# sashajenner/honours

Hardware: AMD Instinct MI355X
Metric: raw-signal MB/s (compress+decompress) (higher is better)
Workload: dtype u16

## Files before the change

honours_amd/csrc/press_abi.hip:

```cpp

#include <dlfcn.h>
#include <stdarg.h>
#include <stdio.h>
#include <stdlib.h>
#include <string.h>

#include <mutex>
#include <thread>
#include <algorithm>
#include <vector>

#include "../../include/press_hip.h"
#include "press_internal.h"
#include "zs_table.h"

using namespace ph;


static thread_local char g_err[256] = "";

static int fail(int code, const char *fmt, ...)
{
	va_list ap;
	va_start(ap, fmt);
// ... 24 lines not shown
	DevBuf() : next(g_bufs) { g_bufs = this; }
	DevBuf(const DevBuf &) = delete;
	DevBuf &operator=(const DevBuf &) = delete;
	int reserve(size_t n)
	{
		if (n <= cap)
			return 0;
		if (p)
			(void) hipFree(p);
		p = nullptr;
		cap = 0;
		size_t want = n + n / 8 + 4096;
		hipError_t e = hipMalloc(&p, want);
		if (e != hipSuccess)
			return fail(PRESS_HIP_EHIP, "hipMalloc(%zu): %s", want, hipGetErrorString(e));
		cap = want;
		return 0;
	}
	void release()
	{
		if (p)
			(void) hipFree(p);
		p = nullptr;
		cap = 0;
	}
};

struct Ctx {
	bool ready = false;
	int device = -1;
	hipStream_t own = nullptr;
	hipStream_t user = nullptr;
	bool use_user = false;
	DevBuf meta, ex_pos, ex_val, low, huff, chunks, gran, ctl, first_chunk, htiles, htrec, hrec, hlist, hread, hwave, hbits, hend, hmin, cbits;
	DevBuf ztmp, zoff, zoff4, zlen, zhist, ztab, zfirst, zblk, zsbits, zbpos, zbflag, zkcnt, zrd, znb, zn, zdcopy, zdhuf, zdunit, zdtree, zdlong, zdctl, zdseq, zdxblk;
	DevBuf sig, off, nsamp, arena, arena_off, lens, lens2, outn, dense, dense_off;
	uint64_t zs_total = 0;
	uint32_t zs_nhost = 0;
	uint32_t *zs_pin = nullptr;
	hipEvent_t zs_ev = nullptr;
	bool have_table = false;
	bool table_trie = false;
	uint32_t tlen[256];
	uint64_t tbits[256];

	hipStream_t stream() const { return use_user ? user : own; }
};

Ctx g;
std::recursive_mutex g_mu;
#define API_LOCK std::lock_guard<std::recursive_mutex> api_lock_(g_mu)
void staging_release();

int ctx_init()
{
	if (g.ready) {
		HIPCHK(hipSetDevice(g.device));
		return 0;
	}
	int ndev = 0;
	hipError_t e = hipGetDeviceCount(&ndev);
	if (e != hipSuccess || ndev == 0)
		return fail(PRESS_HIP_EHIP, "no HIP device: %s", hipGetErrorString(e));
	if (g.device < 0)
		HIPCHK(hipGetDevice(&g.device));
	HIPCHK(hipSetDevice(g.device));
	HIPCHK(hipStreamCreateWithFlags(&g.own, hipStreamNonBlocking));
// ... 333 lines not shown
		    g.zdctl.reserve(sizeof(ZsDCtl)))
			return PRESS_HIP_EHIP;
	}
	if (is_zs(method) && !decode) {
		const size_t mc = max_chunks_of(total_samples, nreads), mb = max_zblocks_of(total_samples, nreads);
		const size_t nr = (size_t) nreads + 1;
		if (g.ztmp.reserve(zs_tmp_bytes(method, total_samples, nreads)) || g.zoff.reserve(nr * 8) || g.zoff4.reserve(nr * 8) ||
		    g.zlen.reserve(nr * 8) || g.zhist.reserve(nr * 1024) || g.ztab.reserve(nr * sizeof(zs::Table)) ||
		    g.zfirst.reserve(nr * 4) || g.zblk.reserve(mb * 4) || g.zsbits.reserve(mb * 16) || g.zbpos.reserve(mb * 4) ||
		    g.zbflag.reserve(mb) || g.zkcnt.reserve(mc * 4) ||
		    g.zrd.reserve(nr * sizeof(ZsRead)) || g.znb.reserve(64) ||
		    g.ex_pos.reserve((total_samples + 64) * 4) || g.ex_val.reserve((total_samples + 64) * 4))
			return PRESS_HIP_EHIP;
	}
	if (is_svb(method) || is_ex(method)) {
		const size_t mc = max_chunks_of(total_samples, nreads);
		if (g.chunks.reserve(mc * sizeof(ChunkDesc)) || g.gran.reserve(2 * mc * sizeof(uint64_t)) ||
		    g.ctl.reserve(2 * sizeof(ChunkCtl)) || g.first_chunk.reserve(((size_t) nreads + 1) * 4))
			return PRESS_HIP_EHIP;
	}
	if (is_ex(method)) {
		if (g.ex_pos.reserve((total_samples + 64) * 4) || g.ex_val.reserve((total_samples + 64) * 4))
			return PRESS_HIP_EHIP;
		if (!decode && is_shuff(method)) {
			const size_t mc = max_chunks_of(total_samples, nreads);
			if (g.cbits.reserve(mc * sizeof(ChunkBits)))
				return PRESS_HIP_EHIP;
		}
		if (is_rc(method) && g.low.reserve(total_samples + 64))
			return PRESS_HIP_EHIP;
		if (decode && is_shuff(method)) {
			const size_t mt = max_htiles_of(total_samples, nreads);
			if (g.low.reserve(total_samples + 64) || g.htiles.reserve(mt * sizeof(HufTile)) ||
			    g.htrec.reserve(mt * sizeof(HufTRec)) || g.hrec.reserve(mt * HUF_HT * 4) ||
			    g.hlist.reserve(hlist_cap_of(mt) * 8) || g.hread.reserve(((size_t) nreads + 1) * 8) ||
			    g.hwave.reserve(mt * (HUF_HT / 64) * 8) || g.hbits.reserve(mt * (HUF_HT / 64) * 8) ||
			    g.hend.reserve(mt * HUF_HT + 64) ||
			    g.hmin.reserve(((size_t) nreads + 1) * 4))
				return PRESS_HIP_EHIP;
		}
	}
	return 0;
}

}


namespace {
constexpr int KT_RING = 128;
struct KTime {
	bool on = false;
	hipEvent_t ev[2][KT_RING][2];
	bool made = false;
	int n[2] = { 0, 0 };
} kt;
}

namespace ph {
static bool kt_muted = false;
void ktime_mute(bool m) { kt_muted = m; }
void ktime_begin(int which, hipStream_t s)
{
	if (kt.on && !kt_muted && kt.n[which] < KT_RING)
		(void) hipEventRecord(kt.ev[which][kt.n[which]][0], s);
}
void ktime_end(int which, hipStream_t s)
{
// ... 650 lines not shown
				       const uint64_t *off, const uint32_t *n, uint64_t total_samples,
				       uint32_t *out_n, int device_resident)
{
	API_LOCK;
	int rc = ctx_init();
	if (rc)
		return rc;
	if ((rc = check_method(method)))
		return rc;
	if (nreads == 0)
		return 0;
	if (!in || !in_off || !in_len || !sig || !off || !n || !out_n)
		return fail(PRESS_HIP_EARG, "NULL argument");
	hipStream_t s = g.stream();
	if ((rc = reserve_scratch(method, total_samples, nreads, true)))
		return rc;
	g.zs_total = total_samples;

	DecodeArgs a;
	memset(&a, 0, sizeof a);
	a.nreads = nreads;
	a.meta = (ReadMeta *) g.meta.p;
	a.ex_pos = (uint32_t *) g.ex_pos.p;
	a.ex_val = (uint32_t *) g.ex_val.p;
	a.low = (uint8_t *) g.low.p;
	a.huff = (const HuffDev *) g.huff.p;
	a.chunks = (ChunkDesc *) g.chunks.p;
	a.gran = (uint64_t *) g.gran.p;
	a.ctl = (ChunkCtl *) g.ctl.p;
	a.first_chunk = (uint32_t *) g.first_chunk.p;
	a.max_chunks = max_chunks_of(total_samples, nreads);
	if (is_shuff(method)) {
		a.htiles = (HufTile *) g.htiles.p;
		a.htrec = (HufTRec *) g.htrec.p;
		a.hrec = (uint32_t *) g.hrec.p;
		a.hlist = (uint32_t *) g.hlist.p;
		a.hread = (uint32_t *) g.hread.p;
		a.hwave = (uint2 *) g.hwave.p;
		a.hbits = (unsigned long long *) g.hbits.p;
		a.hend = (uint8_t *) g.hend.p;
		a.hmin = (uint32_t *) g.hmin.p;
		a.max_htiles = max_htiles_of(total_samples, nreads);
		a.hlist_cap = (uint32_t) hlist_cap_of(a.max_htiles);
		a.huf_minlen = table_minlen() | (g.table_trie ? HUF_NEEDS_TRIE : 0u);
	}

	if (device_resident) {
		if ((uintptr_t) sig & 15)
			return fail(PRESS_HIP_EARG, "sig must be 16-byte aligned");
		a.in = in;
		a.in_off = in_off;
		a.in_len = in_len;
		a.sig = sig;
		a.off = off;
		a.nsamp = n;
		a.out_n = out_n;
		return launch_depress(method, a, s);
	}

	uint64_t dense = 0;
	std::vector<uint64_t> doff(nreads);
	std::vector<Piece> pc;
	pc.reserve(nreads);
	for (uint32_t r = 0; r < nreads; r++) {
		if (off[r] & 7)
			return fail(PRESS_HIP_EARG, "off[%u] is not a multiple of 8 samples", r);
		if (off[r] + n[r] > total_samples)
// ... 602 lines not shown
```

honours_amd/csrc/press_huffman.hip:

```cpp

#include "press_internal.h"
#include "press_packed.h"
#include <cstddef>
#include <type_traits>

namespace ph {

#ifdef HUF_STAMPS
__device__ unsigned long long g_hstamp[32];
#define HSTAMP_DECL                                             \
	unsigned long long hs_t = __builtin_amdgcn_s_memtime(); \
	unsigned long long hs_acc[8] = { 0, 0, 0, 0, 0, 0, 0, 0 }
#define HSTAMP(i)                                                              \
	do {     \
		__builtin_amdgcn_sched_barrier(0);                             \
		const unsigned long long hs_n = __builtin_amdgcn_s_memtime(); \
		hs_acc[(i) & 7] += hs_n - hs_t;                                \
		hs_t = hs_n;                                                   \
		__builtin_amdgcn_sched_barrier(0);                             \
	} while (0)
#define HSTAMP_FLUSH(base)                                                     \
	do {                                                                   \
		if ((threadIdx.x & 63) == 0)                                   \
			for (int hs_i = 0; hs_i < 8; hs_i++)                   \
// ... 503 lines not shown
	load_len_tables(a.huff, &lds.tabs, 64);
	uint32_t *col = img + lane;
	const uint64_t gend = (uint64_t) (k0 + nt) * HT;
	for (uint64_t g = g0; g < gend; g++) {
		const uint32_t k = (uint32_t) (g / HT), tid = (uint32_t) (g % HT);
		const HufTile *dp = a.htiles + k;
		const uint32_t nbits_t = uniform(dp->nbits);
		if ((uint64_t) tid * OWN >= nbits_t)
			break;
		const uint32_t pe = uniform((uint32_t) __hip_atomic_load(a.hend + g - 1, __ATOMIC_RELAXED, __HIP_MEMORY_SCOPE_AGENT));
		const uint32_t rec = uniform(__hip_atomic_load(a.hrec + g, __ATOMIC_RELAXED, __HIP_MEMORY_SCOPE_AGENT));
		if ((rec & 0xFFu) == pe)
			continue;
		wave_lds_sync();
		if (lane == 0)
			col_load<NDW>(col, a.in + dp->src, (int32_t) tid * (OWN / 8), 0, (int32_t) ((nbits_t + 7) >> 3));
		wave_lds_sync();
		uint32_t c2, d2;
		const uint32_t e2 = len_scan<TRIE>(col, &lds.tabs, a.huff, (lane || pe == R_END) ? HEND : pe, OWN,
					     clamp_nb((int64_t) nbits_t - (int64_t) tid * OWN), c2, d2);
		if (lane == 0) {
			a.hrec[g] = pack_rec(pe == R_END ? HEND : pe, c2, d2);
			atomicAdd(reinterpret_cast<unsigned long long *>(a.hwave + (uint64_t) k * (HT / 64) + (tid >> 6)),
				  ((unsigned long long) ((d2 - (rec >> 16)) & 0xFFFFu) << 32) +
					  (unsigned long long) (long long) (int32_t) (c2 - ((rec >> 8) & 0xFFu)));
			__hip_atomic_store(a.hend + g, (uint8_t) (e2 == HEND ? R_END : e2 - OWN), __ATOMIC_RELAXED, __HIP_MEMORY_SCOPE_AGENT);
		}
		__builtin_amdgcn_fence(__ATOMIC_RELEASE, "agent");
	}
}

__device__ __forceinline__ uint32_t unzz16(uint32_t z) { return ((z >> 1) ^ (0u - (z & 1u))) & 0xFFFFu; }

__global__ __launch_bounds__(HT) void k_huf_chain(DecodeArgs a)
{
	__shared__ uint32_t s_w[HT / 64], s_wd[HT / 64];

	const uint32_t r = blockIdx.x;
	const uint32_t tid = threadIdx.x;
	const uint32_t k0 = uniform(a.hread[2 * r]), nt = uniform(a.hread[2 * r + 1]);
	if (!nt)
		return;
	uint64_t cum = 0;
	uint32_t dcum = 0;
	for (uint32_t b = 0; b < nt; b += HT) {
		const uint32_t u = b + tid;
		uint32_t c = 0, dt = 0;
		if (u < nt) {
			const uint4 *wp = reinterpret_cast<const uint4 *>(a.hwave + (uint64_t) (k0 + u) * (HT / 64));
			const uint4 w01 = wp[0], w23 = wp[1];
			c = w01.x + w01.z + w23.x + w23.z;
			dt = (w01.y + w01.w + w23.y + w23.w) & 0xFFFFu;
		}
		const uint32_t inc = wave_scan(c);
		const uint32_t dinc = wave_scan(dt);
		if ((tid & 63) == 63) {
			s_w[tid >> 6] = inc;
			s_wd[tid >> 6] = dinc;
		}
		__syncthreads();
		uint32_t before = 0, total = 0, dbefore = 0, dtotal = 0;
#pragma unroll
		for (int w2 = 0; w2 < HT / 64; w2++) {
			const uint32_t x = s_w[w2], y = s_wd[w2];
			if (w2 < (int) (tid >> 6)) {
				before += x;
				dbefore += y;
			}
			total += x;
			dtotal += y;
		}
		if (u < nt) {
			const uint64_t bs = cum + before + inc - c;
			a.htrec[k0 + u].base = bs > 0xFFFFFFFFull ? 0xFFFFFFFFu : (uint32_t) bs;
			a.htrec[k0 + u].dbase = (dcum + dbefore + dinc - dt) & 0xFFFFu;
		}
		cum += total;
		dcum += dtotal;
		__syncthreads();
	}
	const uint32_t want = uniform(a.htiles[k0].want);
	const uint32_t nlow = cum < want ? (uint32_t) cum : want;
	const uint32_t nex = uniform(a.meta[r].nex);
	const uint64_t o0 = a.htiles[k0].low;
	uint32_t *val = a.ex_val + o0;
	uint32_t xcum = 0;
	for (uint32_t b = 0; b < nex; b += HT) {
		const uint32_t e = b + tid;
		const uint32_t z = e < nex ? (val[e] & 0xFFFFu) : 0u;
		const uint32_t dl = e < nex ? unzz16(z) : 0u;
		const uint32_t inc = wave_scan(dl);
		if ((tid & 63) == 63)
			s_w[tid >> 6] = inc;
		__syncthreads();
		uint32_t before = 0, total = 0;
#pragma unroll
		for (int w2 = 0; w2 < HT / 64; w2++) {
			const uint32_t x = s_w[w2];
			if (w2 < (int) (tid >> 6))
				before += x;
			total += x;
		}
		if (e < nex)
			val[e] = z | (((xcum + before + inc - dl) & 0xFFFFu) << 16);
		xcum += total;
		__syncthreads();
	}
	const bool fused = nlow >= 1 && (nex == 0 || a.ex_pos[o0 + nex - 1] < nlow + nex);
	for (uint32_t u = tid; u < nt; u += HT)
		a.htrec[k0 + u].fused = fused ? 1u : 0u;
	static_assert(HT / 64 == 4, "a tile's wave totals are two 16-byte loads");
	if (tid == 0) {
		a.meta[r].nlow = nlow;
		if (fused)
			a.hread[2 * r + 1] = nt | HUF_FUSED;
	}
}


constexpr uint32_t EMIT_STG = 4096;

template <bool TRIE>
__device__ __forceinline__ void emit_codes(const uint32_t *col_, const uint32_t *lut_, const uint16_t *lut2_,
					   const HuffDev *hd, uint32_t p, uint32_t nmine, uint8_t *wp_)
{
	const lds_cu32p col = (lds_cu32p) col_;
	const lds_cu8p lut = (lds_cu8p) lut_;
	const lds_cu16p lut2 = (lds_cu16p) lut2_;
	auto long_entry = [&](uint32_t e, uint32_t wnd) -> uint32_t {
		if (TRIE && e == 0xFFFFFFFFu) {
			const uint32_t t = trie_code(hd, wnd);
			return t ? ((t & 0xFFFFFF00u) | ((uint32_t) unzz8(t & 0xFFu) & 0xFFu)) : 0u;
		}
		const uint32_t e2 = lut2[(e & 0xFFFu) + ((wnd >> HUF_LUT_BITS) & ((1u << ((e >> 12) & 15u)) - 1u))];
		return e2 == 0xFFFFu ? 0u : (((uint32_t) unzz8(e2 & 0xFFu) & 0xFFu) | (e2 & 0x1F00u) | ((e2 & 0x1F00u) << 16));
	};
	typedef lds_u8p WP;
	WP w = (WP) wp_;
	const WP wend = w + nmine;
	WP wlim = nmine ? wend - 1 : w;
	constexpr uint32_t PB = 30;
	const lds_cu32p colm = col - 64;
	uint32_t pp = p + PB;
	uint32_t jj = pp >> 5;
// ... 10 lines not shown
			w += 1u + ((e >> 29) & 1u);
			pp += (e >> 8) & 0x1Fu;
			const uint32_t jn = pp >> 5;
			if (jn != jj) {
				w0 = w1;
				w1 = w2;
			}
			jj = jn;
		}
	}
	if (w < wend) {
		const uint32_t wnd = __builtin_amdgcn_alignbit(w1, w0, pp);
		uint32_t e = *(lds_cu32p) (lut + (wnd & (((1u << HUF_LUT_BITS) - 1u) << 2)));
		if (e >= HUF_LONG)
			e = long_entry(e, wnd >> 2);
		w[0] = (uint8_t) e;
	}
}


__device__ __forceinline__ uint32_t lower_bound_u32(const uint32_t *p, uint32_t n, uint32_t key)
{
	uint32_t lo = 0, hi = n;
	while (lo < hi) {
		const uint32_t mid = (lo + hi) >> 1;
		if (p[mid] < key)
			lo = mid + 1;
		else
			hi = mid;
	}
	return lo;
}

__device__ __forceinline__ uint32_t keys_below(const uint32_t *pos, uint32_t nex, uint32_t key)
{
	uint32_t lo = 0, hi = nex;
	while (lo < hi) {
		const uint32_t mid = (lo + hi) >> 1;
		if (uniform(pos[mid]) - mid < key)
			lo = mid + 1;
		else
			hi = mid;
	}
	return lo;
}

template <typename LOWAT>
__device__ __forceinline__ void gather8(LOWAT lowat, const uint32_t *pos, const uint32_t *val, uint32_t zd0,
					uint32_t i0, uint32_t Ia, uint32_t Ib, uint32_t e_first, uint32_t e_cnt,
					uint32_t v[4])
{
	v[0] = v[1] = v[2] = v[3] = 0;
	const uint32_t lo = i0 > Ia ? i0 : Ia;
	const uint32_t hi = i0 + 8 < Ib ? i0 + 8 : Ib;
	if (lo >= hi)
		return;
	const uint32_t uf = lo ? lo - 1 : 0;
	const uint32_t e_end = e_first + e_cnt;
	uint32_t e = e_first + lower_bound_u32(pos + e_first, e_cnt, uf);
	uint32_t l = uf - e;
	uint32_t nextpos = e < e_end ? pos[e] : 0xFFFFFFFFu;
#pragma unroll
	for (int h = 0; h < 8; h++) {
		const uint32_t i = i0 + h;
		if (i >= lo && i < hi) {
			uint32_t dl;
			if (i == 0) {
				dl = unzz16(zd0);
			} else if (i - 1 == nextpos) {
				dl = unzz16(val[e] & 0xFFFFu);
				e++;
				nextpos = e < e_end ? pos[e] : 0xFFFFFFFFu;
			} else {
				dl = lowat(l) & 0xFFFFu;
				l++;
			}
			v[h >> 1] |= dl << (16 * (h & 1));
		}
	}
}

struct EmitRead {
	const uint32_t *pos, *val;
	int16_t *out;
	uint32_t nex, zd0, q, nlow;
};

constexpr uint32_t EMIT_ALIGN = 8;

__device__ __forceinline__ void expand8s(uint2 dd, uint32_t v[4])
{
	typedef short i16x2 __attribute__((ext_vector_type(2)));
	const i16x2 eight = { 8, 8 };
	const uint32_t t[4] = { __builtin_amdgcn_perm(0, dd.x, 0x010c000c), __builtin_amdgcn_perm(0, dd.x, 0x030c020c),
				__builtin_amdgcn_perm(0, dd.y, 0x010c000c), __builtin_amdgcn_perm(0, dd.y, 0x030c020c) };
#pragma unroll
	for (int h = 0; h < 4; h++)
		v[h] = __builtin_bit_cast(uint32_t, __builtin_bit_cast(i16x2, t[h]) >> eight);
}

struct EmitPlan {
	uint32_t L0, L1;
	uint32_t Ea, ecnt;
	uint32_t Ia, Ib;
	uint32_t base;
	uint32_t pe;
};

__device__ __forceinline__ EmitPlan emit_plan(const EmitRead &R, uint32_t L0, uint32_t quota, uint32_t B0, uint32_t lane,
					      uint32_t kraw, uint32_t vraw)
{
	const uint32_t key = kraw == 0xFFFFFFFFu ? kraw : kraw - lane;
	EmitPlan P;
	P.L0 = L0;
	P.L1 = L0 + quota;
	const uint32_t nex = R.nex;
	const bool lastw = P.L1 == R.nlow;
	uint32_t Ea = 0, Eb = 0;
	if (nex && nex <= 64) {
		Ea = (uint32_t) __popcll(__ballot(key < P.L0));
		Eb = (uint32_t) __popcll(__ballot(key < P.L1));
	} else if (nex) {
		Ea = keys_below(R.pos, nex, P.L0);
		Eb = keys_below(R.pos, nex, P.L1);
	}
	if (lastw)
		Eb = nex;
	P.Ea = Ea;
	P.ecnt = Eb - Ea;
	P.Ia = L0 ? L0 + Ea + 1 : 0u;
	P.Ib = P.L1 + Eb + 1;
	P.base = 0;
	if (L0) {
		P.base = unzz16(R.zd0) + B0;
		if (Ea) {
			const uint32_t pv = nex <= 64 ? (uint32_t) __builtin_amdgcn_readlane((int) vraw, (int) (Ea - 1)) : uniform(R.val[Ea - 1]);
			P.base += (pv >> 16) + unzz16(pv & 0xFFFFu);
		}
	}
	if (nex <= 64) {
		const uint32_t pl = (uint32_t) __shfl((int) kraw, (int) ((Ea + lane) & 63u), 64);
		P.pe = lane < P.ecnt ? pl : 0xFFFFFFFFu;
	} else {
		P.pe = (P.ecnt <= 64 && lane < P.ecnt) ? R.pos[Ea + lane] : 0xFFFFFFFFu;
	}
	return P;
}

__device__ __forceinline__ void emit_samples16(const uint8_t *src, const EmitRead &R, const EmitPlan &P, uint32_t lane)
{
	const uint32_t L0 = P.L0, L1 = P.L1, Ea = P.Ea, ecnt = P.ecnt, Ia = P.Ia, Ib = P.Ib, pe = P.pe;
	uint32_t base = P.base;
	auto ex_below = [&](uint32_t key) -> uint32_t {
		if (ecnt == 0)
			return 0u;
		if (ecnt <= 64)
			return (uint32_t) __popcll(__ballot(pe < key));
		return uniform(lower_bound_u32(R.pos + Ea, ecnt, key));
	};
	const bool shift = uniform(R.q) != 0;
	const u16x2 qq = { (unsigned short) R.q, (unsigned short) R.q };
	const uint32_t *s32 = reinterpret_cast<const uint32_t *>(src);
	for (uint32_t g = Ia & ~(EMIT_ALIGN - 1); g < Ib; g += 1024) {
		const uint32_t i0 = g + lane * 16;
		const uint32_t e0 = ex_below(g ? g - 1 : 0u), e1 = ex_below(g + 1023);
		const bool plain = e0 == e1 && g != 0;
		const bool ragged = g < Ia || g + 1024 > Ib;
		uint32_t v[8];
		if (plain) {
			const bool any = i0 + 16 > Ia && i0 < Ib;
			const int32_t o = any ? (int32_t) (i0 - 1 - Ea - e0 - L0) : 0;
			const int32_t j = o >> 2;
			const uint32_t sh = (uint32_t) (o & 3) * 8u;
			const uint32_t d0 = s32[j], d1 = s32[j + 1], d2 = s32[j + 2], d3 = s32[j + 3], d4 = s32[j + 4];
			uint2 da = make_uint2(__builtin_amdgcn_alignbit(d1, d0, sh), __builtin_amdgcn_alignbit(d2, d1, sh));
			uint2 db = make_uint2(__builtin_amdgcn_alignbit(d3, d2, sh), __builtin_amdgcn_alignbit(d4, d3, sh));
			if (g < Ia) {
				auto mask8 = [&](uint2 &dd, uint32_t ia) {
					const uint32_t lo = Ia > ia ? (Ia - ia < 8 ? Ia - ia : 8u) : 0u;
					const uint64_t m = lo >= 8 ? 0ull : ~((1ull << (8 * lo)) - 1ull);
					dd.x &= (uint32_t) m;
					dd.y &= (uint32_t) (m >> 32);
				};
				mask8(da, i0);
				mask8(db, i0 + 8);
			}
			expand8s(da, v);
			expand8s(db, v + 4);
		} else {
			auto lowat = [&](uint32_t l) -> uint32_t { return (l >= L0 && l < L1) ? (uint32_t) (int32_t) (int8_t) src[l - L0] : 0u; };
			gather8(lowat, R.pos, R.val, R.zd0, i0, Ia, Ib, Ea, ecnt, v);
			gather8(lowat, R.pos, R.val, R.zd0, i0 + 8, Ia, Ib, Ea, ecnt, v + 4);
			__builtin_amdgcn_s_waitcnt(0x0F70);
		}
		const uint32_t ta = lane_prefix8(v) & 0xFFFFu;
		const uint32_t tb = lane_prefix8(v + 4) & 0xFFFFu;
		const uint32_t tot = (ta + tb) & 0xFFFFu;
		const uint32_t inc = wave_incl_scan_dpp(tot);
		const uint32_t ba = (base + inc - tot) & 0xFFFFu, bb = (ba + ta) & 0xFFFFu;
		const uint32_t ba2 = ba | (ba << 16), bb2 = bb | (bb << 16);
#pragma unroll
		for (int h = 0; h < 4; h++) {
			v[h] = pk_add16(v[h], ba2);
			v[4 + h] = pk_add16(v[4 + h], bb2);
		}
		if (shift) {
#pragma unroll
			for (int h = 0; h < 8; h++)
				v[h] = __builtin_bit_cast(uint32_t, __builtin_bit_cast(u16x2, v[h]) << qq);
		}
#if defined(EMIT_ABL) && EMIT_ABL == 1
		if (R.nlow == 0x7FFFFFFFu)
#endif
#pragma unroll
		for (int hh = 0; hh < 2; hh++) {
			const uint32_t ia = i0 + 8 * hh;
			if (!ragged || (ia >= Ia && ia + 8 <= Ib)) {
				typedef uint32_t u32x4 __attribute__((ext_vector_type(4)));
				const u32x4 vv = { v[4 * hh], v[4 * hh + 1], v[4 * hh + 2], v[4 * hh + 3] };
#ifdef EMIT_NT_STORES
				__builtin_nontemporal_store(vv, reinterpret_cast<u32x4 *>(R.out + ia));
#else
				*reinterpret_cast<u32x4 *>(R.out + ia) = vv;
#endif
			} else if (ia < Ib && ia + 8 > Ia) {
#pragma unroll
				for (uint32_t h = 0; h < 8; h++)
					if (ia + h >= Ia && ia + h < Ib)
						R.out[ia + h] = (int16_t) (v[4 * hh + (h >> 1)] >> (16 * (h & 1)));
			}
		}
		base += (uint32_t) __builtin_amdgcn_readlane((int) inc, 63);
	}
}

__device__ __forceinline__ uint32_t zz_bytes(uint32_t d)
{
	return ((d << 1) & 0xFEFEFEFEu) ^ (((d >> 7) & 0x01010101u) * 0xFFu);
}

#ifndef EMIT_WG
#define EMIT_WG 512
#endif
#ifndef EMIT_PER_CU
#define EMIT_PER_CU 2
// ... 40 lines not shown
		s_chunk[threadIdx.x] = ~0ull;
	{
		const uint4 *s4 = reinterpret_cast<const uint4 *>(a.huff->lut32);
		uint4 *d4 = reinterpret_cast<uint4 *>(lut);
		for (uint32_t i = threadIdx.x; i < (1u << HUF_LUT_BITS) / 4; i += WGE)
			d4[i] = s4[i];
		const uint4 *t4 = reinterpret_cast<const uint4 *>(a.huff->lut2);
		uint4 *u4 = reinterpret_cast<uint4 *>(lut2);
		for (uint32_t i = threadIdx.x; i < (uint32_t) HUF_L2_ENTRIES / 8; i += WGE)
			u4[i] = t4[i];
	}
	uint32_t *col = img[wv] + lane;
	uint8_t *stg = stg_all.s[wv];
	__syncthreads();
	auto draw = [&]() -> uint32_t {
		uint32_t u = 0;
		if (lane == 0) {
			const uint32_t t = atomicAdd(&s_ticket, 1u);
			const uint32_t c = t / EMIT_UC, slot = t % EMIT_UC;
			unsigned long long *cs = &s_chunk[c & 63u];
			if (slot == 0) {
				u = atomicAdd(&a.ctl->units, EMIT_UC);
				__hip_atomic_store(cs, ((unsigned long long) c << 32) | u, __ATOMIC_RELAXED, __HIP_MEMORY_SCOPE_WORKGROUP);
			} else {
				unsigned long long v;
				do {
					v = __hip_atomic_load(cs, __ATOMIC_RELAXED, __HIP_MEMORY_SCOPE_WORKGROUP);
				} while ((uint32_t) (v >> 32) != c);
				u = (uint32_t) v + slot;
			}
		}
		return uniform(u);
	};
	static_assert(sizeof(HufTile) == 32 && sizeof(HufTRec) == 32 && sizeof(ReadMeta) == 32 && offsetof(HufTile, nbits) == 16 &&
			      offsetof(HufTile, read) == 24 && offsetof(HufTRec, base) == 8 && offsetof(HufTRec, fused) == 28,
		      "the records are read as eight dwords each");
	auto fetch_tile = [&](uint32_t u) -> uint32_t {
		uint32_t v = 0;
		if (u < nunits && lane < 24) {
			const uint32_t k = u / (HT / 64);
			const uint32_t *p = lane < 8 ? reinterpret_cast<const uint32_t *>(a.htiles + k)
					  : lane < 16 ? reinterpret_cast<const uint32_t *>(a.htrec + k)
						      : reinterpret_cast<const uint32_t *>(a.hwave + (uint64_t) k * (HT / 64));
			v = p[lane & 7];
		}
		return v;
	};
	struct Unit {
		uint32_t u, nbits_t, read, want, fused, cb, db, base, dbase;
		uint64_t srco, roff;
	};
	auto resolve = [&](uint32_t u, uint32_t tv) -> Unit {
		auto at = [&](int i) -> uint32_t { return (uint32_t) __builtin_amdgcn_readlane((int) tv, i); };
		Unit U;
		U.u = u;
		U.srco = ((uint64_t) at(1) << 32) | at(0);
		U.roff = ((uint64_t) at(3) << 32) | at(2);
		U.nbits_t = at(4);
		U.read = at(6);
		U.want = at(7);
		U.base = at(8 + 2);
		U.dbase = at(8 + 3);
		U.fused = at(8 + 7);
		const uint32_t wq = u % (HT / 64);
		U.cb = (wq > 0 ? at(16) : 0u) + (wq > 1 ? at(18) : 0u) + (wq > 2 ? at(20) : 0u);
		U.db = (wq > 0 ? at(17) : 0u) + (wq > 1 ? at(19) : 0u) + (wq > 2 ? at(21) : 0u);
		return U;
	};
	struct Stage2 {
		uint32_t pay[NDW];
		uint32_t rec;
		uint4 m0, m1;
		bool fast;
	};
	auto issue2 = [&](const Unit &U, Stage2 &S) {
		const uint32_t tid = (U.u % (HT / 64)) * 64 + lane;
		const int32_t rb0 = (int32_t) tid * (OWN / 8), nby = (int32_t) ((U.nbits_t + 7) >> 3);
		S.fast = !any64(rb0 + 4 * NDW > nby);
		const uint8_t *q = a.in + U.srco + rb0;
		if (S.fast) {
			uint4 t[NDW / 4 ? NDW / 4 : 1];
#pragma unroll
			for (int j = 0; j < NDW / 4; j++)
				t[j] = ld16_pay(q + 16 * j);
#pragma unroll
			for (int j = 0; j < NDW % 4; j++)
				S.pay[NDW / 4 * 4 + j] = ld4_pay(q + 4 * (NDW / 4 * 4 + j));
#pragma unroll
			for (int j = 0; j < NDW / 4; j++) {
				S.pay[4 * j + 0] = t[j].x;
				S.pay[4 * j + 1] = t[j].y;
				S.pay[4 * j + 2] = t[j].z;
				S.pay[4 * j + 3] = t[j].w;
			}
		}
		S.rec = a.hrec[(uint64_t) (U.u / (HT / 64)) * HT + tid];
		const uint4 *mp = reinterpret_cast<const uint4 *>(a.meta + U.read);
		S.m0 = mp[0];
		S.m1 = mp[1];
	};
	auto land2 = [&](const Unit &U, const Stage2 &S) {
		wave_lds_sync();
		if (S.fast) {
#pragma unroll
			for (int j = 0; j < NDW; j++)
				col[j * 64] = S.pay[j];
		} else {
			const uint32_t tid = (U.u % (HT / 64)) * 64 + lane;
			col_load<NDW>(col, a.in + U.srco, (int32_t) tid * (OWN / 8), 0, (int32_t) ((U.nbits_t + 7) >> 3));
		}
		wave_lds_sync();
	};
	HSTAMP_DECL;
	const uint32_t u_first = draw();
	if (u_first >= nunits)
		return;
	Unit U = resolve(u_first, fetch_tile(u_first)), Un = {}, Unn = {};
	Stage2 S, Sn = {};
	issue2(U, S);
	land2(U, S);
	uint32_t u_nxt = draw();
	if (u_nxt < nunits)
		Un = resolve(u_nxt, fetch_tile(u_nxt));
	for (;;) {
		const uint32_t u_nn = draw();
		const uint32_t tv_nn = fetch_tile(u_nn);
		const bool more = u_nxt < nunits;
		if (more)
			issue2(Un, Sn);
		HSTAMP(0);
		const uint32_t tid = (U.u % (HT / 64)) * 64 + lane;
		const uint32_t rec = S.rec;
		const uint32_t want = U.want;
		const uint64_t roff = U.roff;
		uint8_t *low = a.low + roff;
		const uint32_t cnt = (rec >> 8) & 0xFFu;
		const uint32_t inc = wave_scan(cnt);
		const uint64_t obase = (uint64_t) U.base + U.cb;
		const uint32_t B0 = U.dbase + (U.db & 0xFFFFu);
		const bool fused = U.fused != 0;
		const uint32_t wsum = uniform((uint32_t) __shfl((int) inc, 63, 64));
		const uint32_t quota = obase >= want ? 0u : (wsum < want - (uint32_t) obase ? wsum : want - (uint32_t) obase);
		const uint32_t ex = inc - cnt;
		const uint32_t f = rec & 0xFFu;
		const uint32_t p0 = f == R_END ? 0u : f;
		uint32_t nmine = (ex >= quota || f == R_END) ? 0u : (cnt < quota - ex ? cnt : quota - ex);
		nmine = ex >= EMIT_STG ? 0u : (nmine < EMIT_STG - ex ? nmine : EMIT_STG - ex);
		uint8_t *dst = low + obase;
		EmitRead R = {};
		if (fused) {
			R.pos = a.ex_pos + roff;
			R.val = a.ex_val + roff;
			R.out = a.sig + roff;
			R.nex = uniform(S.m0.x);
			R.zd0 = uniform(S.m0.z);
			R.q = uniform(S.m0.w);
			R.nlow = uniform(S.m1.z);
		}
		(void) tid;
		const uint32_t kraw = (fused && quota && lane < R.nex) ? R.pos[lane] : 0xFFFFFFFFu;
		const uint32_t vraw = (fused && quota && lane < R.nex) ? R.val[lane] : 0u;
		HSTAMP(2);
		{
#if defined(EMIT_ABL) && EMIT_ABL == 3
			if (a.nreads == 0x7FFFFFFFu)
#endif
			emit_codes<TRIE>(col, lut, lut2, a.huff, p0, nmine, stg + ex);
			HSTAMP(3);
			if (more)
				land2(Un, Sn);
			else
				wave_lds_sync();
			if (u_nn < nunits)
				Unn = resolve(u_nn, tv_nn);
			HSTAMP(1);
			if (fused) {
				if (quota) {
					const EmitPlan P = emit_plan(R, (uint32_t) obase, quota, B0, lane, kraw, vraw);
					HSTAMP(4);
#if defined(EMIT_ABL) && EMIT_ABL == 2
					if (a.nreads == 0x7FFFFFFFu)
#endif
					emit_samples16(stg, R, P, lane);
					HSTAMP(5);
				}
			} else {
				for (uint32_t o = lane * 16; o < quota; o += 64 * 16) {
					uint4 v = *reinterpret_cast<const uint4 *>(stg + o);
					v = make_uint4(zz_bytes(v.x), zz_bytes(v.y), zz_bytes(v.z), zz_bytes(v.w));
					if (o + 16 <= quota) {
						__builtin_memcpy(dst + o, &v, 16);
					} else {
						const uint32_t vv[4] = { v.x, v.y, v.z, v.w };
						for (uint32_t b = 0; o + b < quota; b++)
							dst[o + b] = (uint8_t) (vv[b >> 2] >> (8 * (b & 3)));
					}
				}
			}
			wave_lds_sync();
		}
		HSTAMP(6);
		if (!more)
			break;
		U = Un;
		S = Sn;
		Un = Unn;
		u_nxt = u_nn;
	}
	HSTAMP_FLUSH(8);
}


constexpr uint32_t TILES_RPW = 16;
__global__ __launch_bounds__(64) void k_huff_tiles(DecodeArgs a)
{
	const uint32_t lane = threadIdx.x;
	const uint32_t r = lane < TILES_RPW ? blockIdx.x * TILES_RPW + lane : 0xFFFFFFFFu;
	const uint32_t minlen = a.huff->minlen, maxlen = a.huff->maxlen;
	const uint32_t OWN = minlen >= 4 ? 256u : minlen >= 2 ? 128u : 64u;
// ... 62 lines not shown

#ifndef HUF_FIX_ROUNDS
#define HUF_FIX_ROUNDS 4
#endif
#ifdef HUF_STAMPS
}
extern "C" int press_hip_huf_stamps(unsigned long long *dst, uint32_t nwords)
{
	unsigned long long z[32] = { 0 };
	if (hipDeviceSynchronize() != hipSuccess ||
	    hipMemcpyFromSymbol(dst, HIP_SYMBOL(ph::g_hstamp), (nwords < 32 ? nwords : 32) * 8) != hipSuccess ||
	    hipMemcpyToSymbol(HIP_SYMBOL(ph::g_hstamp), z, sizeof z) != hipSuccess)
		return -1;
	return 0;
}
namespace ph {
#endif

constexpr int HUF_FIX_LAUNCHES = HUF_FIX_ROUNDS;

template <int RU, bool TRIE>
static void run_huff_decode(const DecodeArgs &a, hipStream_t s)
{
	const uint32_t nt = a.max_htiles ? a.max_htiles : 1;
	const uint32_t ngs = (nt * (HT / 64) + WGS / 64 - 1) / (WGS / 64);
	const uint32_t grid = ngs < HUF_SYNC_PER_CU * 256u ? ngs : HUF_SYNC_PER_CU * 256u;
	const uint32_t nge = (nt * (HT / 64) + WGE / 64 - 1) / (WGE / 64);
	const uint32_t ge = nge < EMIT_PER_CU * 256u ? nge : EMIT_PER_CU * 256u;
	hipLaunchKernelGGL((k_huf_sync<RU, TRIE>), dim3(grid), dim3(WGS), 0, s, a);
	hipLaunchKernelGGL(k_huf_list, dim3((nt * (HT / 64) + LIST_WG - 1) / LIST_WG), dim3(LIST_WG), 0, s, a);
	for (int round = 0; round < HUF_FIX_LAUNCHES; round++)
		hipLaunchKernelGGL((k_huf_fix<RU, TRIE>), dim3(FIX_WG >= 1024 ? 512 : FIX_WG >= 512 ? 768 : 1280), dim3(FIX_WG), 0, s, a, round, round + 1 == HUF_FIX_LAUNCHES ? 1 : 0);
	hipLaunchKernelGGL((k_huf_serial<RU, TRIE>), dim3(a.nreads), dim3(64), 0, s, a);
	hipLaunchKernelGGL(k_huf_chain, dim3(a.nreads), dim3(HT), 0, s, a);
	hipLaunchKernelGGL((k_huf_emit<RU, TRIE>), dim3(ge), dim3(WGE), 0, s, a);
}

template <int RU>
static void run_huff_decode_t(const DecodeArgs &a, bool trie, hipStream_t s)
{
	if (trie)
		run_huff_decode<RU, true>(a, s);
	else
		run_huff_decode<RU, false>(a, s);
}

void launch_huff_decode(const DecodeArgs &a0, uint32_t minlen, hipStream_t s)
{
	const bool trie = (minlen & HUF_NEEDS_TRIE) != 0;
	minlen &= ~HUF_NEEDS_TRIE;
	DecodeArgs a = a0;
	a.ctl = a0.ctl + 1;
	hipLaunchKernelGGL(k_huff_tiles, dim3((a.nreads + TILES_RPW - 1) / TILES_RPW), dim3(64), 0, s, a);
	if (minlen >= 4)
		run_huff_decode_t<128>(a, trie, s);
	else if (minlen >= 2)
		run_huff_decode_t<64>(a, trie, s);
	else
		run_huff_decode_t<32>(a, trie, s);
}

}
```

honours_amd/csrc/press_internal.h:

```cpp
#pragma once

#include <hip/hip_runtime.h>
#include <stdint.h>

namespace ph {

enum ExFmt : int {
	EXF_VBE21 = 0,
	EXF_VBBE21 = 1,
	EXF_VBSBE21 = 2,
	EXF_VBSSE21 = 3,
	EXF_EXZD = 4
};

struct ReadMeta {
	uint32_t nex;
	uint32_t ored;
	uint32_t zd0;
	uint32_t q;
	uint32_t hdr;
	uint32_t seclen;
	uint32_t nlow;
	uint32_t status;
};

constexpr int HUF_LUT_BITS = 12;
constexpr int HUF_L2_ENTRIES = 3072;
constexpr int HUF_L2_IDS = 64;
struct HuffDev {
	uint32_t enc[256];
	uint16_t lut[1 << HUF_LUT_BITS];
	int16_t child[1024][2];
	int16_t leaf[1024];
	uint32_t minlen, maxlen;
	uint16_t lut2[HUF_L2_ENTRIES];
	uint16_t l2off[256];
	uint8_t l2bits[256];
	alignas(16) uint32_t lut32[1 << HUF_LUT_BITS];
	alignas(16) uint32_t mlut[1 << HUF_LUT_BITS];
	alignas(16) uint16_t l2ld[HUF_L2_ENTRIES];
	alignas(16) uint32_t alut[1 << HUF_LUT_BITS];
	alignas(16) uint16_t flut[1 << HUF_LUT_BITS];
};
constexpr uint32_t HUF_A_CNT = 9, HUF_A_SUM = 16;
constexpr uint32_t HUF_NEEDS_TRIE = 0x80000000u;
constexpr uint32_t HUF_L2_NONE = HUF_L2_ENTRIES - 1;
constexpr uint32_t HUF_MLONG = 1u << 31;
constexpr uint32_t HUF_M_MAXN = 8;
constexpr uint32_t HUF_LONG = 1u << 30;
constexpr uint32_t HUF_TWO = 1u << 29;

constexpr int HUF_HT = 256;
struct HufTRec {
	uint32_t rsv0[2];
	uint32_t base;
	uint32_t dbase;
	uint32_t rsv1[3];
	uint32_t fused;
};
static_assert(sizeof(HufTRec) == 32, "HufTRec");
constexpr uint32_t HUF_FUSED = 0x80000000u;

constexpr uint32_t CHUNK = 32768;
struct ChunkDesc {
	uint64_t sig_off;
	uint64_t out_base;
	uint32_t n;
	uint32_t j;
	uint32_t read;
	uint32_t cap_ok;
	uint64_t ebefore;
	uint32_t ecnt[4];
	uint16_t kmask[4];
};
static_assert(sizeof(ChunkDesc) == 64, "ChunkDesc is one 64-byte line");
struct ChunkBits {
	uint64_t before;
	uint32_t q[4];
	uint32_t pad[2];
};
struct ChunkCtl {
	uint32_t ticket;
	uint32_t pad0[31];
	uint32_t nchunks;
	uint32_t pad1[31];
	uint32_t ticket2;
	uint32_t pad2[31];
	uint32_t lists[32];
	uint32_t units;
	uint32_t pad4[31];
	uint32_t sunits;
	uint32_t pad5[31];
};
// ... 20 lines not shown
	uint32_t *zhist;
	uint32_t *zkcnt;
};

struct HufTile {
	uint64_t src;
	uint64_t low;
	uint32_t nbits;
	uint32_t t_last;
	uint32_t read;
	uint32_t want;
};

struct DecodeArgs {
	const uint8_t *in;
	const uint64_t *in_off;
	const uint64_t *in_len;
	int16_t *sig;
	const uint64_t *off;
	const uint32_t *nsamp;
	uint32_t *out_n;
	ReadMeta *meta;
	uint32_t *ex_pos;
	uint32_t *ex_val;
	uint8_t *low;
	const HuffDev *huff;
	uint32_t nreads;
	ChunkDesc *chunks;
	uint64_t *gran;
	ChunkCtl *ctl;
	uint32_t *first_chunk;
	uint32_t max_chunks;
	HufTile *htiles;
	HufTRec *htrec;
	uint32_t *hrec;
	uint32_t *hlist;
	uint8_t *hend;
	uint32_t *hmin;
	uint32_t *hread;
	uint2 *hwave;
	unsigned long long *hbits;
	uint32_t max_htiles;
	uint32_t hlist_cap;
	uint32_t huf_minlen;
};

struct ZsRead {
	uint32_t nk, nd;
	uint32_t knz;
	uint32_t mode;
	uint32_t dbase;
	uint32_t plen;
	uint32_t pad[2];
};
struct ZsCopy {
	uint64_t src, dst;
	uint32_t n, fill;
};
struct ZsHuf {
	uint64_t src, dst;
	uint32_t cs, R;
	uint32_t four;
	uint32_t pad;
};
struct ZsUnit {
	uint32_t read, tree, count, pad;
};
// ... 81 lines not shown
```

Baseline: 766,800.

## Precompute per-wave emit plans in chain kernel as compact HufUnit records

The chain kernel now writes one 32-byte HufUnit per 64-lane wave unit rather than per-tile base records. Each record holds the source offset, output base, quota, byte count, zigzag base, fused flag and exception range, with the exception bounds found by a per-thread dual binary search. The emit kernel then reads eight dwords per unit instead of gathering tile, trec, wave and meta records and computing the plan with ballots or binary searches in its hot loop. In exchange the chain kernel does an extra pass summing wave counts through a shared atomic and does per-unit searches, and fields are packed into narrow bitfields with fixed width limits.

```diff
diff --git a/honours_amd/csrc/press_abi.hip b/honours_amd/csrc/press_abi.hip
--- a/honours_amd/csrc/press_abi.hip
+++ b/honours_amd/csrc/press_abi.hip
@@ -80,7 +80,7 @@
 	hipStream_t own = nullptr;
 	hipStream_t user = nullptr;
 	bool use_user = false;
-	DevBuf meta, ex_pos, ex_val, low, huff, chunks, gran, ctl, first_chunk, htiles, htrec, hrec, hlist, hread, hwave, hbits, hend, hmin, cbits;
+	DevBuf meta, ex_pos, ex_val, low, huff, chunks, gran, ctl, first_chunk, htiles, hunit, hrec, hlist, hread, hwave, hbits, hend, hmin, cbits;
 	DevBuf ztmp, zoff, zoff4, zlen, zhist, ztab, zfirst, zblk, zsbits, zbpos, zbflag, zkcnt, zrd, znb, zn, zdcopy, zdhuf, zdunit, zdtree, zdlong, zdctl, zdseq, zdxblk;
 	DevBuf sig, off, nsamp, arena, arena_off, lens, lens2, outn, dense, dense_off;
 	uint64_t zs_total = 0;
@@ -480,7 +480,7 @@
 		if (decode && is_shuff(method)) {
 			const size_t mt = max_htiles_of(total_samples, nreads);
 			if (g.low.reserve(total_samples + 64) || g.htiles.reserve(mt * sizeof(HufTile)) ||
-			    g.htrec.reserve(mt * sizeof(HufTRec)) || g.hrec.reserve(mt * HUF_HT * 4) ||
+			    g.hunit.reserve(mt * (HUF_HT / 64) * sizeof(HufUnit)) || g.hrec.reserve(mt * HUF_HT * 4) ||
 			    g.hlist.reserve(hlist_cap_of(mt) * 8) || g.hread.reserve(((size_t) nreads + 1) * 8) ||
 			    g.hwave.reserve(mt * (HUF_HT / 64) * 8) || g.hbits.reserve(mt * (HUF_HT / 64) * 8) ||
 			    g.hend.reserve(mt * HUF_HT + 64) ||
@@ -1197,7 +1197,7 @@
 	a.max_chunks = max_chunks_of(total_samples, nreads);
 	if (is_shuff(method)) {
 		a.htiles = (HufTile *) g.htiles.p;
-		a.htrec = (HufTRec *) g.htrec.p;
+		a.hunit = (HufUnit *) g.hunit.p;
 		a.hrec = (uint32_t *) g.hrec.p;
 		a.hlist = (uint32_t *) g.hlist.p;
 		a.hread = (uint32_t *) g.hread.p;
diff --git a/honours_amd/csrc/press_huffman.hip b/honours_amd/csrc/press_huffman.hip
--- a/honours_amd/csrc/press_huffman.hip
+++ b/honours_amd/csrc/press_huffman.hip
@@ -559,58 +559,51 @@
 
 __device__ __forceinline__ uint32_t unzz16(uint32_t z) { return ((z >> 1) ^ (0u - (z & 1u))) & 0xFFFFu; }
 
+__device__ __forceinline__ void keys_below2(const uint32_t *pos, uint32_t nex, uint32_t ka, uint32_t kb, uint32_t &ea, uint32_t &eb)
+{
+	uint32_t la = 0, lb = 0;
+	for (uint32_t step = nex ? 1u << (31 - __builtin_clz(nex)) : 0u; step; step >>= 1) {
+		const uint32_t ia = la + step - 1, ib = lb + step - 1;
+		const uint32_t pa = ia < nex ? pos[ia] : 0u, pb = ib < nex ? pos[ib] : 0u;
+		if (ia < nex && pa - ia < ka)
+			la += step;
+		if (ib < nex && pb - ib < kb)
+			lb += step;
+	}
+	ea = la;
+	eb = lb;
+}
+
+template <int RU>
 __global__ __launch_bounds__(HT) void k_huf_chain(DecodeArgs a)
 {
+	constexpr uint32_t UB = 64 * HufGeo<RU>::OWN / 8;
+	constexpr uint32_t UPT = HT / 64;
 	__shared__ uint32_t s_w[HT / 64], s_wd[HT / 64];
+	__shared__ unsigned long long s_cum;
 
 	const uint32_t r = blockIdx.x;
 	const uint32_t tid = threadIdx.x;
 	const uint32_t k0 = uniform(a.hread[2 * r]), nt = uniform(a.hread[2 * r + 1]);
 	if (!nt)
 		return;
-	uint64_t cum = 0;
-	uint32_t dcum = 0;
-	for (uint32_t b = 0; b < nt; b += HT) {
-		const uint32_t u = b + tid;
-		uint32_t c = 0, dt = 0;
-		if (u < nt) {
-			const uint4 *wp = reinterpret_cast<const uint4 *>(a.hwave + (uint64_t) (k0 + u) * (HT / 64));
-			const uint4 w01 = wp[0], w23 = wp[1];
-			c = w01.x + w01.z + w23.x + w23.z;
-			dt = (w01.y + w01.w + w23.y + w23.w) & 0xFFFFu;
-		}
-		const uint32_t inc = wave_scan(c);
-		const uint32_t dinc = wave_scan(dt);
-		if ((tid & 63) == 63) {
-			s_w[tid >> 6] = inc;
-			s_wd[tid >> 6] = dinc;
-		}
-		__syncthreads();
-		uint32_t before = 0, total = 0, dbefore = 0, dtotal = 0;
-#pragma unroll
-		for (int w2 = 0; w2 < HT / 64; w2++) {
-			const uint32_t x = s_w[w2], y = s_wd[w2];
-			if (w2 < (int) (tid >> 6)) {
-				before += x;
-				dbefore += y;
-			}
-			total += x;
-			dtotal += y;
-		}
-		if (u < nt) {
-			const uint64_t bs = cum + before + inc - c;
-			a.htrec[k0 + u].base = bs > 0xFFFFFFFFull ? 0xFFFFFFFFu : (uint32_t) bs;
-			a.htrec[k0 + u].dbase = (dcum + dbefore + dinc - dt) & 0xFFFFu;
-		}
-		cum += total;
-		dcum += dtotal;
-		__syncthreads();
+	const uint32_t nu = nt * UPT;
+	const uint2 *hw = a.hwave + (uint64_t) k0 * UPT;
+	if (tid == 0)
+		s_cum = 0;
+	__syncthreads();
+	{
+		uint64_t c = 0;
+		for (uint32_t u = tid; u < nu; u += HT)
+			c += hw[u].x;
+		if (c)
+			atomicAdd(&s_cum, (unsigned long long) c);
 	}
 	const uint32_t want = uniform(a.htiles[k0].want);
-	const uint32_t nlow = cum < want ? (uint32_t) cum : want;
 	const uint32_t nex = uniform(a.meta[r].nex);
 	const uint64_t o0 = a.htiles[k0].low;
 	uint32_t *val = a.ex_val + o0;
+	const uint32_t *pos = a.ex_pos + o0;
 	uint32_t xcum = 0;
 	for (uint32_t b = 0; b < nex; b += HT) {
 		const uint32_t e = b + tid;
@@ -633,10 +626,73 @@
 		xcum += total;
 		__syncthreads();
 	}
-	const bool fused = nlow >= 1 && (nex == 0 || a.ex_pos[o0 + nex - 1] < nlow + nex);
-	for (uint32_t u = tid; u < nt; u += HT)
-		a.htrec[k0 + u].fused = fused ? 1u : 0u;
-	static_assert(HT / 64 == 4, "a tile's wave totals are two 16-byte loads");
+	__syncthreads();
+	const uint64_t cumall = s_cum;
+	const uint32_t nlow = cumall < want ? (uint32_t) cumall : want;
+	const bool fused = nlow >= 1 && (nex == 0 || pos[nex - 1] < nlow + nex);
+	const uint32_t zd0 = uniform(a.meta[r].zd0) & 0xFFFFu, q = uniform(a.meta[r].q);
+	const uint64_t src0 = a.htiles[k0].src;
+	const int64_t nby0 = (int64_t) ((a.htiles[k0].nbits + 7u) >> 3);
+	uint64_t cum = 0;
+	uint32_t dcum = 0;
+	for (uint32_t b = 0; b < nu; b += HT) {
+		const uint32_t u = b + tid;
+		uint32_t c = 0, dt = 0;
+		if (u < nu) {
+			const uint2 w = hw[u];
+			c = w.x;
+			dt = w.y & 0xFFFFu;
+		}
+		const uint32_t inc = wave_scan(c);
+		const uint32_t dinc = wave_scan(dt);
+		if ((tid & 63) == 63) {
+			s_w[tid >> 6] = inc;
+			s_wd[tid >> 6] = dinc;
+		}
+		__syncthreads();
+		uint32_t before = 0, total = 0, dbefore = 0, dtotal = 0;
+#pragma unroll
+		for (int w2 = 0; w2 < HT / 64; w2++) {
+			const uint32_t x = s_w[w2], y = s_wd[w2];
+			if (w2 < (int) (tid >> 6)) {
+				before += x;
+				dbefore += y;
+			}
+			total += x;
+			dtotal += y;
+		}
+		if (u < nu) {
+			const uint64_t ob = cum + before + inc - c;
+			const uint32_t L0 = ob > 0xFFFFFFFFull ? 0xFFFFFFFFu : (uint32_t) ob;
+			const uint32_t quota = L0 >= want ? 0u : (c < want - L0 ? c : want - L0);
+			const uint32_t L1 = L0 + quota;
+			uint32_t Ea = 0, Eb = 0;
+			if (fused && quota) {
+				keys_below2(pos, nex, L0, L1, Ea, Eb);
+				if (L1 == nlow)
+					Eb = nex;
+			}
+			uint32_t bz = zd0;
+			if (L0) {
+				bz = unzz16(zd0) + ((dcum + dbefore + dinc - dt) & 0xFFFFu);
+				if (Ea) {
+					const uint32_t pv = val[Ea - 1];
+					bz += (pv >> 16) + unzz16(pv & 0xFFFFu);
+				}
+				bz &= 0xFFFFu;
+			}
+			const uint64_t src = src0 + (uint64_t) u * UB;
+			const int64_t nby = nby0 - (int64_t) u * UB;
+			const uint32_t nbyc = nby <= 0 ? 0u : (nby > (int64_t) HUF_U_NBY ? HUF_U_NBY : (uint32_t) nby);
+			uint4 *d = reinterpret_cast<uint4 *>(a.hunit + (uint64_t) k0 * UPT + u);
+			d[0] = make_uint4((uint32_t) src, (uint32_t) (src >> 32) | (bz << 16), (uint32_t) o0, (uint32_t) (o0 >> 32));
+			d[1] = make_uint4(L0, quota | (nbyc << 14) | ((q & 15u) << 26) | (fused ? 1u << 30 : 0u), Ea, Eb - Ea);
+		}
+		cum += total;
+		dcum += dtotal;
+		__syncthreads();
+	}
+	static_assert(HUF_U_QUOTA >= 64u * 255u, "a unit's quota");
 	if (tid == 0) {
 		a.meta[r].nlow = nlow;
 		if (fused)
@@ -713,19 +769,6 @@
 	return lo;
 }
 
-__device__ __forceinline__ uint32_t keys_below(const uint32_t *pos, uint32_t nex, uint32_t key)
-{
-	uint32_t lo = 0, hi = nex;
-	while (lo < hi) {
-		const uint32_t mid = (lo + hi) >> 1;
-		if (uniform(pos[mid]) - mid < key)
-			lo = mid + 1;
-		else
-			hi = mid;
-	}
-	return lo;
-}
-
 template <typename LOWAT>
 __device__ __forceinline__ void gather8(LOWAT lowat, const uint32_t *pos, const uint32_t *val, uint32_t zd0,
 					uint32_t i0, uint32_t Ia, uint32_t Ib, uint32_t e_first, uint32_t e_cnt,
@@ -764,7 +807,7 @@
 struct EmitRead {
 	const uint32_t *pos, *val;
 	int16_t *out;
-	uint32_t nex, zd0, q, nlow;
+	uint32_t zd0, q;
 };
 
 constexpr uint32_t EMIT_ALIGN = 8;
@@ -787,46 +830,6 @@
 	uint32_t base;
 	uint32_t pe;
 };
-
-__device__ __forceinline__ EmitPlan emit_plan(const EmitRead &R, uint32_t L0, uint32_t quota, uint32_t B0, uint32_t lane,
-					      uint32_t kraw, uint32_t vraw)
-{
-	const uint32_t key = kraw == 0xFFFFFFFFu ? kraw : kraw - lane;
-	EmitPlan P;
-	P.L0 = L0;
-	P.L1 = L0 + quota;
-	const uint32_t nex = R.nex;
-	const bool lastw = P.L1 == R.nlow;
-	uint32_t Ea = 0, Eb = 0;
-	if (nex && nex <= 64) {
-		Ea = (uint32_t) __popcll(__ballot(key < P.L0));
-		Eb = (uint32_t) __popcll(__ballot(key < P.L1));
-	} else if (nex) {
-		Ea = keys_below(R.pos, nex, P.L0);
-		Eb = keys_below(R.pos, nex, P.L1);
-	}
-	if (lastw)
-		Eb = nex;
-	P.Ea = Ea;
-	P.ecnt = Eb - Ea;
-	P.Ia = L0 ? L0 + Ea + 1 : 0u;
-	P.Ib = P.L1 + Eb + 1;
-	P.base = 0;
-	if (L0) {
-		P.base = unzz16(R.zd0) + B0;
-		if (Ea) {
-			const uint32_t pv = nex <= 64 ? (uint32_t) __builtin_amdgcn_readlane((int) vraw, (int) (Ea - 1)) : uniform(R.val[Ea - 1]);
-			P.base += (pv >> 16) + unzz16(pv & 0xFFFFu);
-		}
-	}
-	if (nex <= 64) {
-		const uint32_t pl = (uint32_t) __shfl((int) kraw, (int) ((Ea + lane) & 63u), 64);
-		P.pe = lane < P.ecnt ? pl : 0xFFFFFFFFu;
-	} else {
-		P.pe = (P.ecnt <= 64 && lane < P.ecnt) ? R.pos[Ea + lane] : 0xFFFFFFFFu;
-	}
-	return P;
-}
 
 __device__ __forceinline__ void emit_samples16(const uint8_t *src, const EmitRead &R, const EmitPlan &P, uint32_t lane)
 {
@@ -891,7 +894,7 @@
 				v[h] = __builtin_bit_cast(uint32_t, __builtin_bit_cast(u16x2, v[h]) << qq);
 		}
 #if defined(EMIT_ABL) && EMIT_ABL == 1
-		if (R.nlow == 0x7FFFFFFFu)
+		if (R.q == 0x7FFFFFFFu)
 #endif
 #pragma unroll
 		for (int hh = 0; hh < 2; hh++) {
@@ -998,51 +1001,43 @@
 		}
 		return uniform(u);
 	};
-	static_assert(sizeof(HufTile) == 32 && sizeof(HufTRec) == 32 && sizeof(ReadMeta) == 32 && offsetof(HufTile, nbits) == 16 &&
-			      offsetof(HufTile, read) == 24 && offsetof(HufTRec, base) == 8 && offsetof(HufTRec, fused) == 28,
-		      "the records are read as eight dwords each");
-	auto fetch_tile = [&](uint32_t u) -> uint32_t {
+	static_assert(offsetof(HufUnit, obase) == 16 && offsetof(HufUnit, ecnt) == 28, "the plan is read as eight dwords");
+	static_assert(63 * (OWN / 8) + 4 * NDW <= HUF_U_NBY, "HufUnit::qnf's byte count tells whether every lane's bytes lie inside");
+	auto fetch_unit = [&](uint32_t u) -> uint32_t {
 		uint32_t v = 0;
-		if (u < nunits && lane < 24) {
-			const uint32_t k = u / (HT / 64);
-			const uint32_t *p = lane < 8 ? reinterpret_cast<const uint32_t *>(a.htiles + k)
-					  : lane < 16 ? reinterpret_cast<const uint32_t *>(a.htrec + k)
-						      : reinterpret_cast<const uint32_t *>(a.hwave + (uint64_t) k * (HT / 64));
-			v = p[lane & 7];
-		}
+		if (u < nunits && lane < 8)
+			v = reinterpret_cast<const uint32_t *>(a.hunit + u)[lane];
 		return v;
 	};
 	struct Unit {
-		uint32_t u, nbits_t, read, want, fused, cb, db, base, dbase;
+		uint32_t u, obase, quota, nby, fused, q, bz, ea, ecnt;
 		uint64_t srco, roff;
 	};
 	auto resolve = [&](uint32_t u, uint32_t tv) -> Unit {
 		auto at = [&](int i) -> uint32_t { return (uint32_t) __builtin_amdgcn_readlane((int) tv, i); };
 		Unit U;
 		U.u = u;
-		U.srco = ((uint64_t) at(1) << 32) | at(0);
+		const uint32_t hb = at(1), qnf = at(5);
+		U.srco = ((uint64_t) (hb & 0xFFFFu) << 32) | at(0);
+		U.bz = hb >> 16;
 		U.roff = ((uint64_t) at(3) << 32) | at(2);
-		U.nbits_t = at(4);
-		U.read = at(6);
-		U.want = at(7);
-		U.base = at(8 + 2);
-		U.dbase = at(8 + 3);
-		U.fused = at(8 + 7);
-		const uint32_t wq = u % (HT / 64);
-		U.cb = (wq > 0 ? at(16) : 0u) + (wq > 1 ? at(18) : 0u) + (wq > 2 ? at(20) : 0u);
-		U.db = (wq > 0 ? at(17) : 0u) + (wq > 1 ? at(19) : 0u) + (wq > 2 ? at(21) : 0u);
+		U.obase = at(4);
+		U.quota = qnf & HUF_U_QUOTA;
+		U.nby = (qnf >> 14) & HUF_U_NBY;
+		U.q = (qnf >> 26) & 15u;
+		U.fused = qnf >> 30;
+		U.ea = at(6);
+		U.ecnt = at(7);
 		return U;
 	};
 	struct Stage2 {
 		uint32_t pay[NDW];
-		uint32_t rec;
-		uint4 m0, m1;
+		uint32_t rec, pe;
 		bool fast;
 	};
 	auto issue2 = [&](const Unit &U, Stage2 &S) {
-		const uint32_t tid = (U.u % (HT / 64)) * 64 + lane;
-		const int32_t rb0 = (int32_t) tid * (OWN / 8), nby = (int32_t) ((U.nbits_t + 7) >> 3);
-		S.fast = !any64(rb0 + 4 * NDW > nby);
+		const int32_t rb0 = (int32_t) lane * (OWN / 8);
+		S.fast = U.nby >= 63 * (OWN / 8) + 4 * NDW;
 		const uint8_t *q = a.in + U.srco + rb0;
 		if (S.fast) {
 			uint4 t[NDW / 4 ? NDW / 4 : 1];
@@ -1060,10 +1055,8 @@
 				S.pay[4 * j + 3] = t[j].w;
 			}
 		}
-		S.rec = a.hrec[(uint64_t) (U.u / (HT / 64)) * HT + tid];
-		const uint4 *mp = reinterpret_cast<const uint4 *>(a.meta + U.read);
-		S.m0 = mp[0];
-		S.m1 = mp[1];
+		S.rec = a.hrec[(uint64_t) U.u * 64 + lane];
+		S.pe = (U.ecnt <= 64 && lane < U.ecnt) ? a.ex_pos[U.roff + U.ea + lane] : 0xFFFFFFFFu;
 	};
 	auto land2 = [&](const Unit &U, const Stage2 &S) {
 		wave_lds_sync();
@@ -1072,8 +1065,7 @@
 			for (int j = 0; j < NDW; j++)
 				col[j * 64] = S.pay[j];
 		} else {
-			const uint32_t tid = (U.u % (HT / 64)) * 64 + lane;
-			col_load<NDW>(col, a.in + U.srco, (int32_t) tid * (OWN / 8), 0, (int32_t) ((U.nbits_t + 7) >> 3));
+			col_load<NDW>(col, a.in + U.srco, (int32_t) lane * (OWN / 8), 0, (int32_t) U.nby);
 		}
 		wave_lds_sync();
 	};
@@ -1081,51 +1073,32 @@
 	const uint32_t u_first = draw();
 	if (u_first >= nunits)
 		return;
-	Unit U = resolve(u_first, fetch_tile(u_first)), Un = {}, Unn = {};
+	Unit U = resolve(u_first, fetch_unit(u_first)), Un = {}, Unn = {};
 	Stage2 S, Sn = {};
 	issue2(U, S);
 	land2(U, S);
 	uint32_t u_nxt = draw();
 	if (u_nxt < nunits)
-		Un = resolve(u_nxt, fetch_tile(u_nxt));
+		Un = resolve(u_nxt, fetch_unit(u_nxt));
 	for (;;) {
 		const uint32_t u_nn = draw();
-		const uint32_t tv_nn = fetch_tile(u_nn);
+		const uint32_t tv_nn = fetch_unit(u_nn);
 		const bool more = u_nxt < nunits;
 		if (more)
 			issue2(Un, Sn);
 		HSTAMP(0);
-		const uint32_t tid = (U.u % (HT / 64)) * 64 + lane;
 		const uint32_t rec = S.rec;
-		const uint32_t want = U.want;
+		const uint32_t quota = U.quota;
+		const uint32_t obase = U.obase;
 		const uint64_t roff = U.roff;
-		uint8_t *low = a.low + roff;
 		const uint32_t cnt = (rec >> 8) & 0xFFu;
 		const uint32_t inc = wave_scan(cnt);
-		const uint64_t obase = (uint64_t) U.base + U.cb;
-		const uint32_t B0 = U.dbase + (U.db & 0xFFFFu);
 		const bool fused = U.fused != 0;
-		const uint32_t wsum = uniform((uint32_t) __shfl((int) inc, 63, 64));
-		const uint32_t quota = obase >= want ? 0u : (wsum < want - (uint32_t) obase ? wsum : want - (uint32_t) obase);
 		const uint32_t ex = inc - cnt;
 		const uint32_t f = rec & 0xFFu;
 		const uint32_t p0 = f == R_END ? 0u : f;
 		uint32_t nmine = (ex >= quota || f == R_END) ? 0u : (cnt < quota - ex ? cnt : quota - ex);
 		nmine = ex >= EMIT_STG ? 0u : (nmine < EMIT_STG - ex ? nmine : EMIT_STG - ex);
-		uint8_t *dst = low + obase;
-		EmitRead R = {};
-		if (fused) {
-			R.pos = a.ex_pos + roff;
-			R.val = a.ex_val + roff;
-			R.out = a.sig + roff;
-			R.nex = uniform(S.m0.x);
-			R.zd0 = uniform(S.m0.z);
-			R.q = uniform(S.m0.w);
-			R.nlow = uniform(S.m1.z);
-		}
-		(void) tid;
-		const uint32_t kraw = (fused && quota && lane < R.nex) ? R.pos[lane] : 0xFFFFFFFFu;
-		const uint32_t vraw = (fused && quota && lane < R.nex) ? R.val[lane] : 0u;
 		HSTAMP(2);
 		{
 #if defined(EMIT_ABL) && EMIT_ABL == 3
@@ -1133,6 +1106,7 @@
 #endif
 			emit_codes<TRIE>(col, lut, lut2, a.huff, p0, nmine, stg + ex);
 			HSTAMP(3);
+			const uint32_t pe = S.pe;
 			if (more)
 				land2(Un, Sn);
 			else
@@ -1142,7 +1116,21 @@
 			HSTAMP(1);
 			if (fused) {
 				if (quota) {
-					const EmitPlan P = emit_plan(R, (uint32_t) obase, quota, B0, lane, kraw, vraw);
+					EmitRead R;
+					R.pos = a.ex_pos + roff;
+					R.val = a.ex_val + roff;
+					R.out = a.sig + roff;
+					R.zd0 = U.bz;
+					R.q = U.q;
+					EmitPlan P;
+					P.L0 = obase;
+					P.L1 = obase + quota;
+					P.Ea = U.ea;
+					P.ecnt = U.ecnt;
+					P.Ia = obase ? obase + U.ea + 1 : 0u;
+					P.Ib = P.L1 + U.ea + U.ecnt + 1;
+					P.base = obase ? U.bz : 0u;
+					P.pe = pe;
 					HSTAMP(4);
 #if defined(EMIT_ABL) && EMIT_ABL == 2
 					if (a.nreads == 0x7FFFFFFFu)
@@ -1151,6 +1139,7 @@
 					HSTAMP(5);
 				}
 			} else {
+				uint8_t *dst = a.low + roff + obase;
 				for (uint32_t o = lane * 16; o < quota; o += 64 * 16) {
 					uint4 v = *reinterpret_cast<const uint4 *>(stg + o);
 					v = make_uint4(zz_bytes(v.x), zz_bytes(v.y), zz_bytes(v.z), zz_bytes(v.w));
@@ -1279,7 +1268,7 @@
 	for (int round = 0; round < HUF_FIX_LAUNCHES; round++)
 		hipLaunchKernelGGL((k_huf_fix<RU, TRIE>), dim3(FIX_WG >= 1024 ? 512 : FIX_WG >= 512 ? 768 : 1280), dim3(FIX_WG), 0, s, a, round, round + 1 == HUF_FIX_LAUNCHES ? 1 : 0);
 	hipLaunchKernelGGL((k_huf_serial<RU, TRIE>), dim3(a.nreads), dim3(64), 0, s, a);
-	hipLaunchKernelGGL(k_huf_chain, dim3(a.nreads), dim3(HT), 0, s, a);
+	hipLaunchKernelGGL(k_huf_chain<RU>, dim3(a.nreads), dim3(HT), 0, s, a);
 	hipLaunchKernelGGL((k_huf_emit<RU, TRIE>), dim3(ge), dim3(WGE), 0, s, a);
 }
 
diff --git a/honours_amd/csrc/press_internal.h b/honours_amd/csrc/press_internal.h
--- a/honours_amd/csrc/press_internal.h
+++ b/honours_amd/csrc/press_internal.h
@@ -51,14 +51,16 @@
 constexpr uint32_t HUF_TWO = 1u << 29;
 
 constexpr int HUF_HT = 256;
-struct HufTRec {
-	uint32_t rsv0[2];
-	uint32_t base;
-	uint32_t dbase;
-	uint32_t rsv1[3];
-	uint32_t fused;
-};
-static_assert(sizeof(HufTRec) == 32, "HufTRec");
+struct HufUnit {
+	uint32_t src_lo;
+	uint32_t src_hi_bz;
+	uint64_t roff;
+	uint32_t obase;
+	uint32_t qnf;
+	uint32_t ea, ecnt;
+};
+static_assert(sizeof(HufUnit) == 32, "HufUnit");
+constexpr uint32_t HUF_U_QUOTA = 0x3FFFu, HUF_U_NBY = 0xFFFu;
 constexpr uint32_t HUF_FUSED = 0x80000000u;
 
 constexpr uint32_t CHUNK = 32768;
@@ -145,7 +147,7 @@
 	uint32_t *first_chunk;
 	uint32_t max_chunks;
 	HufTile *htiles;
-	HufTRec *htrec;
+	HufUnit *hunit;
 	uint32_t *hrec;
 	uint32_t *hlist;
 	uint8_t *hend;
```

After: 782,000 (median of 6 runs). 1.02x the previous value.
